# shibatch/rectdetect

Hardware: AMD Instinct MI355X
Metric: 1920x1080 frames/sec (higher is better)
Workload: dtype u8/i32/f32 (bit-exact integer + IEEE f32 stencil path)

## Files before the change

### rectdetect_amd/csrc/rd_k_label.hip

```cpp
#include <stdlib.h>
#include "rd_device.h"
#include "rd_kernels.h"
#include "rd_tidy_tile.h"

namespace {

using namespace rd;

inline int cdiv(int a, int b) { return (a + b - 1) / b; }
const dim3 block2(64, 4);
inline dim3 grid2(int iw, int ih) { return dim3(cdiv(iw, 64), cdiv(ih, 4)); }

#define LT_W 64
#ifndef LT_H
#define LT_H 32
#endif
__device__ __forceinline__ int lt_ld(const int *lab, int a) { return __hip_atomic_load(lab + a, __ATOMIC_RELAXED, __HIP_MEMORY_SCOPE_WORKGROUP); }
__device__ __forceinline__ int lt_find(const int *lab, int a) {
  int l = lt_ld(lab, a);
  while (l != a) { a = l; l = lt_ld(lab, a); }
  return a;
}
__device__ __forceinline__ void lt_union(int *lab, int a, int b) {
  for (;;) {
    a = lt_find(lab, a);
    b = lt_find(lab, b);
    if (a == b) return;
    if (a < b) { const int t = a; a = b; b = t; }
    const int old = atomicMin(&lab[a], b);
    if (old == a) return;
    a = old;
  }
}

#ifndef LT_TY
#define LT_TY 4
#endif
#ifndef LT_TY1
#define LT_TY1 LT_TY
#endif
#define LT_MP 68
template <int SRC, int TY>
__global__ __launch_bounds__(64 * TY) void k_label_tile(int *__restrict__ label, const int *__restrict__ pix, int bgc, int iw, int ih, int *__restrict__ pix_out,
                                                    const float *__restrict__ nms, int *__restrict__ mask0, int *__restrict__ zero_plane, size_t zs, int gdim) {
  constexpr bool BOUNDARY = SRC == 1;
  const rd_tile rd_b = rd_block_tile(gdim);
  if (rd_b.x < 0) return;
  RD_ZSHIFTZ(rd_b.z, zs, label, pix, pix_out, nms, mask0, zero_plane);
  __shared__ int lab[LT_W * LT_H];
  __shared__ int pv[LT_W * LT_H];
  const int tx = threadIdx.x, x = rd_b.x * LT_W + tx, y0 = rd_b.y * LT_H;
  const bool xin = x < iw;
  int v00;
  bool uniform = true;
  int pv8[LT_H / TY];
  if constexpr (SRC == 2) {
    __shared__ __align__(16) uint8_t A[(LT_H + 2 * TD_M) * TD_P], B[(LT_H + 2 * TD_M) * TD_P];
    rect_tidy_tile<LT_H>(A, B, rd_b.x * LT_W, y0, threadIdx.y * 64 + tx, nms, mask0, pix_out, zero_plane, iw, ih, pv8);
    __shared__ int s_t00;
    if (threadIdx.y == 0 && tx == 0) s_t00 = pv8[0];
    __syncthreads();
    v00 = s_t00;
  } else if constexpr (SRC == 3) {
#pragma unroll
    for (int k = 0; k < LT_H / TY; k++) {
      const int y = y0 + threadIdx.y + k * TY;
      const bool in = xin && y < ih;
      const float e = nms[in ? y * iw + x : 0];
      pv8[k] = e > 0.0f ? 1 : 0;
      if (in) { pix_out[y * iw + x] = pv8[k]; zero_plane[y * iw + x] = 0; }
    }
    v00 = nms[(size_t)y0 * iw + rd_b.x * LT_W] > 0.0f ? 1 : 0;
  } else if constexpr (!BOUNDARY) {
    v00 = pix[(size_t)y0 * iw + rd_b.x * LT_W];
#pragma unroll
    for (int k = 0; k < LT_H / TY; k++) {
      const int y = y0 + threadIdx.y + k * TY;
      pv8[k] = pix[(xin && y < ih) ? y * iw + x : 0];
    }
  } else {
    __shared__ int t[(LT_H + 4) * LT_MP];
    __shared__ uint8_t hu[(LT_H + 4) * 64];
    const int x0 = rd_b.x * LT_W, tid = threadIdx.y * 64 + tx;
    const int r00 = pix[(size_t)y0 * iw + x0];
    bool flat = true;
    {
      constexpr int NR = (LT_H + 4 + TY - 1) / TY;
      static_assert(LT_MP == 68 && 4 * (LT_H + 4) <= 64 * TY, "four columns beyond the lanes, one cell per thread");
      int v[NR + 1];
      bool ok[NR + 1];
      const int xl = x0 - 2 + tx;
      const bool cok = xl >= 0 && xl < iw;
#pragma unroll
      for (int i = 0; i < NR; i++) {
        const int r = threadIdx.y + TY * i, yy = y0 - 2 + r;
        ok[i] = r < LT_H + 4 && cok && yy >= 0 && yy < ih;
        v[i] = pix[ok[i] ? yy * iw + xl : 0];
      }
      const int sr = tid >> 2, sc = 64 + (tid & 3);
      {
        const int xx = x0 - 2 + sc, yy = y0 - 2 + sr;
        ok[NR] = sr < LT_H + 4 && xx < iw && yy >= 0 && yy < ih;
        v[NR] = pix[ok[NR] ? yy * iw + xx : 0];
      }
#pragma unroll
      for (int i = 0; i < NR; i++) {
        const int r = threadIdx.y + TY * i;
        if (r < LT_H + 4) { flat = flat && (!ok[i] || v[i] == r00); t[r * LT_MP + tx] = ok[i] ? v[i] : 0; }
      }
      if (sr < LT_H + 4) { flat = flat && (!ok[NR] || v[NR] == r00); t[sr * LT_MP + sc] = ok[NR] ? v[NR] : 0; }
    }
    if (__syncthreads_and(flat)) {
#pragma unroll
      for (int k = 0; k < LT_H / TY; k++) {
        const int y = y0 + threadIdx.y + k * TY;
        if (xin && y < ih) { pix_out[y * iw + x] = -1; label[y * iw + x] = -1; }
      }
      return;
    }
    for (int r = threadIdx.y; r < LT_H + 4; r += TY) {
      const int *row = t + r * LT_MP + tx + 2;
      const int c = row[0];
      hu[r * 64 + tx] = (row[-2] == c && row[-1] == c && row[1] == c && row[2] == c) ? 1 : 0;
    }
    __syncthreads();
#pragma unroll
    for (int k = 0; k < LT_H / TY; k++) {
      const int r = threadIdx.y + k * TY;
      const int y = y0 + r;
      int res = -1;
      if (xin && y < ih && x > 1 && y > 1 && x < iw - 2 && y < ih - 2) {
        const int c0 = t[(r + 2) * LT_MP + tx + 2];
        bool same = true;
#pragma unroll
        for (int dy = 0; dy < 5; dy++) same = same && t[(r + dy) * LT_MP + tx + 2] == c0 && hu[(r + dy) * 64 + tx] != 0;
        if (!same) res = c0;
      }
      pv8[k] = res;
      if (xin && y < ih) pix_out[y * iw + x] = res;
    }
    __shared__ int s_v00;
    if (threadIdx.y == 0 && tx == 0) s_v00 = pv8[0];
    __syncthreads();
    v00 = s_v00;
  }
#pragma unroll
  for (int k = 0; k < LT_H / TY; k++) {
    const int r = threadIdx.y + k * TY;
    const int y = y0 + r;
    const bool valid = xin && y < ih;
    const int v = valid ? pv8[k] : 0;
    uniform = uniform && (!valid || v == v00);
    const int vl = __shfl_up(v, 1);
    const bool lvalid = __shfl_up((int)valid, 1) != 0;
    const bool same = valid && tx > 0 && lvalid && vl == v;
    const unsigned long long starts = __ballot(!same);
    const unsigned long long upto = starts & ((2ull << tx) - 1ull);
    const int start = 63 - __clzll((long long)upto);
    pv[r * LT_W + tx] = v;
    lab[r * LT_W + tx] = (!valid || v == bgc) ? -1 : r * LT_W + start;
  }
  {
    if (__syncthreads_and(uniform)) {
      const int l = v00 == bgc ? -1 : y0 * iw + rd_b.x * LT_W;
#pragma unroll
      for (int r = threadIdx.y; r < LT_H; r += TY) {
        const int y = y0 + r;
        if (xin && y < ih) label[y * iw + x] = l;
      }
      return;
    }
  }
#pragma unroll
  for (int r = threadIdx.y; r < LT_H; r += TY) {
    if (r == 0) continue;
    const int q = r * LT_W + tx;
    if (lab[q] < 0) continue;
    const int v = pv[q];
    const bool wSame = tx > 0 && lab[q - 1] >= 0 && pv[q - 1] == v;
    const bool nSame = lab[q - LT_W] >= 0 && pv[q - LT_W] == v;
    const bool nwSame = tx > 0 && lab[q - LT_W - 1] >= 0 && pv[q - LT_W - 1] == v;
    if (nSame) {
      if (!(wSame && nwSame)) lt_union(lab, q, q - LT_W);
    } else {
      const bool neSame = tx < LT_W - 1 && lab[q - LT_W + 1] >= 0 && pv[q - LT_W + 1] == v;
      const bool eSame = tx < LT_W - 1 && lab[q + 1] >= 0 && pv[q + 1] == v;
      if (nwSame && !wSame) lt_union(lab, q, q - LT_W - 1);
      if (neSame && !eSame) lt_union(lab, q, q - LT_W + 1);
    }
  }
  __syncthreads();
#pragma unroll
  for (int r = threadIdx.y; r < LT_H; r += TY) {
    const int y = y0 + r;
    if (!xin || y >= ih) continue;
    const int q = r * LT_W + tx;
    int l = lab[q];
    if (l >= 0) { l = lt_find(lab, l); l = (y0 + l / LT_W) * iw + rd_b.x * LT_W + l % LT_W; }
    label[y * iw + x] = l;
  }
}

#define LB_SEEN 512
#ifndef LB_DEDUPE
#define LB_DEDUPE 1
#endif
__device__ __forceinline__ void border_union(int *label, int la, int lb, bool want, unsigned long long *seen = nullptr) {
  if (!want) { la = -1; lb = -2; }
  const int pa = __shfl_up(la, 1), pb = __shfl_up(lb, 1);
  bool mine = want && !(__lane_id() > 0 && pa == la && pb == lb);
  if (mine && seen != nullptr) {
    const unsigned long long key = ((unsigned long long)(unsigned)la << 32) | (unsigned)lb;
    unsigned h = ((unsigned)la * 2654435761u ^ (unsigned)lb * 40503u) >> 23;
    for (int probe = 0; probe < 4; probe++) {
      const unsigned long long was = atomicCAS(&seen[h], ~0ull, key);
      if (was == key) { mine = false; break; }
      if (was == ~0ull) break;
      h = (h + 1) & (LB_SEEN - 1);
    }
  }
  if (mine) {
    int a = la, b = lb;
    for (;;) {
      int na = ld_agent(label + a), nb = ld_agent(label + b);
      while (na != a || nb != b) { a = na; b = nb; na = ld_agent(label + a); nb = ld_agent(label + b); }
      if (a == b) break;
      if (a < b) { const int t = a; a = b; b = t; }
      const int old = atomicMin(&label[a], b);
      if (old == a) break;
      a = old;
    }
    const int r = a < b ? a : b;
    if (r < la) atomicMin(&label[la], r);
    if (r < lb) atomicMin(&label[lb], r);
  }
}

__global__ __launch_bounds__(256) void k_label_border(int *label, const int *__restrict__ pix, int bgc, int iw, int ih, int hblocks, size_t zs) {
  RD_ZSHIFT(zs, label, pix);
#if LB_DEDUPE
  __shared__ unsigned long long seen_tab[LB_SEEN];
  for (int i = threadIdx.x; i < LB_SEEN; i += 256) seen_tab[i] = ~0ull;
  __syncthreads();
  unsigned long long *const seen = seen_tab;
#else
  unsigned long long *const seen = nullptr;
#endif
  const bool horizontal = (int)blockIdx.x < hblocks;
  const int t = (horizontal ? blockIdx.x : blockIdx.x - hblocks) * blockDim.x + threadIdx.x;
  if (horizontal) {
    const int nb = (ih - 1) / LT_H;
    const int x = t % iw, k = t / iw;
    const bool in = k < nb;
    const int y = (k + 1) * LT_H;
    const int p = y * iw + x;
    const int v = in ? pix[p] : bgc;
    const bool act = in && v != bgc;
    const bool wSame = act && x > 0 && pix[p - 1] == v;
    const bool nSame = act && pix[p - iw] == v;
    const bool nwSame = act && x > 0 && pix[p - iw - 1] == v;
    const bool neSame = act && x < iw - 1 && pix[p - iw + 1] == v;
    const bool eSame = act && x < iw - 1 && pix[p + 1] == v;
    const int pc = in ? p : 0;
    const int l0 = label[pc], ln = label[in ? p - iw : 0], lnw = label[(in && x > 0) ? p - iw - 1 : 0], lne = label[(in && x < iw - 1) ? p - iw + 1 : 0];
    border_union(label, l0, ln, nSame && !(wSame && nwSame), seen);
    border_union(label, l0, lnw, !nSame && nwSame && !wSame, seen);
    border_union(label, l0, lne, !nSame && neSame && !eSame, seen);
  } else {
    const int nb = (iw - 1) / LT_W;
    const int y = t % ih, k = t / ih;
    const bool in = k < nb;
    const int x = (k + 1) * LT_W;
    const int p = y * iw + x;
    const int v = in ? pix[p] : bgc;
    const bool act = in && v != bgc;
    const bool wSame = act && pix[p - 1] == v;
    const bool nSame = act && y > 0 && pix[p - iw] == v;
    const bool nwSame = act && y > 0 && pix[p - iw - 1] == v;
    const int pc = in ? p : 0;
    const int l0 = label[pc], lw = label[in ? p - 1 : 0], lnw = label[(in && y > 0) ? p - iw - 1 : 0];
    const int ll0 = label[in ? p - 1 : 0], llne = label[(in && y > 0) ? p - 1 - iw + 1 : 0];
    border_union(label, l0, lw, wSame, seen);
    border_union(label, l0, lnw, nwSame && !nSame && !wSame, seen);
    const int pl = p - 1;
    const int vl = in ? pix[pl] : bgc;
    const bool actl = in && vl != bgc && y > 0;
    const bool lne = actl && pix[pl - iw + 1] == vl;
    const bool ln = actl && pix[pl - iw] == vl;
    const bool le = actl && pix[pl + 1] == vl;
    border_union(label, ll0, llne, lne && !ln && !le, seen);
  }
}

__global__ __launch_bounds__(256) void k_label_flatten(int *label, int n, int *vt_table, int *vt_claim, int *vt_list, size_t zs) {
  RD_ZSHIFT(zs, label, vt_table, vt_claim, vt_list);
  const int stride = gridDim.x * blockDim.x;
  for (int i0 = blockIdx.x * blockDim.x + threadIdx.x; i0 < n; i0 += stride * 4) {
    int l[4];
#pragma unroll
    for (int k = 0; k < 4; k++) { const int i = i0 + k * stride; l[k] = i < n ? label[i] : -1; }
    int r[4], n[4];
#pragma unroll
    for (int k = 0; k < 4; k++) { r[k] = l[k] < 0 ? 0 : l[k]; n[k] = l[k] < 0 ? 0 : label[r[k]]; }
    while ((n[0] != r[0]) | (n[1] != r[1]) | (n[2] != r[2]) | (n[3] != r[3])) {
#pragma unroll
      for (int k = 0; k < 4; k++) { r[k] = n[k]; const int v = label[r[k]]; n[k] = l[k] < 0 ? 0 : v; }
    }
#pragma unroll
    for (int k = 0; k < 4; k++)
      if (l[k] >= 0 && r[k] != l[k]) label[i0 + k * stride] = r[k];
  }
  if (vt_list != nullptr && blockIdx.x == 0) {
    const int m = vt_list[0];
    for (int j = threadIdx.x; j < m; j += blockDim.x) {
      const int slot = vt_list[1 + j];
      int *e = vt_table + (size_t)slot * 5;
      e[0] = 0; e[1] = 0; e[2] = 0; e[3] = 0; e[4] = 0;
      vt_claim[slot] = 0x7f7f7f7f;
    }
    __syncthreads();
    if (threadIdx.x == 0) vt_list[0] = 0;
  }
}

#define CS_ROWS 4
#define CS_T 1024
__global__ __launch_bounds__(256) void k_calc_strength(int *out, const float *__restrict__ edge, int *label, int iw, int ih, const int8_t *__restrict__ add, int flatten, size_t zs) {
  RD_ZSHIFT(zs, out, edge, label);
  __shared__ int keys[CS_T], vals[CS_T];
  const int tid = threadIdx.y * 64 + threadIdx.x;
  for (int t = tid; t < CS_T; t += 256) { keys[t] = -1; vals[t] = 0; }
  const int x = blockIdx.x * 64 + threadIdx.x, yb = blockIdx.y * (4 * CS_ROWS) + threadIdx.y;
  int ls[CS_ROWS], as[CS_ROWS];
  float es[CS_ROWS];
#pragma unroll
  for (int k = 0; k < CS_ROWS; k++) {
    const int y = yb + 4 * k;
    const int p = (x < iw && y < ih) ? y * iw + x : 0;
    ls[k] = label[p];
    es[k] = edge[p];
    as[k] = add != nullptr ? add[p] : 0;
  }
  if (flatten) {
    int r[CS_ROWS], n[CS_ROWS];
    bool act[CS_ROWS];
#pragma unroll
    for (int k = 0; k < CS_ROWS; k++) { act[k] = x < iw && yb + 4 * k < ih && ls[k] >= 0; r[k] = act[k] ? ls[k] : 0; }
#pragma unroll
    for (int k = 0; k < CS_ROWS; k++) n[k] = act[k] ? label[r[k]] : 0;
    for (;;) {
      bool moving = false;
#pragma unroll
      for (int k = 0; k < CS_ROWS; k++) moving = moving || n[k] != r[k];
      if (!moving) break;
#pragma unroll
      for (int k = 0; k < CS_ROWS; k++) { r[k] = n[k]; const int v = label[r[k]]; n[k] = act[k] ? v : 0; }
    }
#pragma unroll
    for (int k = 0; k < CS_ROWS; k++)
      if (act[k] && r[k] != ls[k]) { label[(yb + 4 * k) * iw + x] = r[k]; ls[k] = r[k]; }
  }
  __syncthreads();
#pragma unroll
  for (int k = 0; k < CS_ROWS; k++) {
    const int y = yb + 4 * k;
    if (x < iw && y < ih && as[k] != 0) atomicAdd(&out[y * iw + x], as[k]);
    int l = -1, val = 0;
    if (x > 0 && y > 0 && x < iw - 1 && y < ih - 1) {
      l = ls[k];
      if (l > 0) { const float e = es[k]; val = (int)(e * e * 10000.0f); }
    }
    if (l > 0 && val != 0) {
      unsigned h = ((unsigned)l * 2654435761u) >> 22;
      int probes = 0;
      for (;;) {
        const int kprev = atomicCAS(&keys[h], -1, l);
        if (kprev == -1 || kprev == l) { atomicAdd(&vals[h], val); break; }
        h = (h + 1) & (CS_T - 1);
        if (++probes == 32) { atomicAdd(&out[l], val); break; }
      }
    }
  }
  __syncthreads();
  for (int t = tid; t < CS_T; t += 256) if (keys[t] != -1 && vals[t] != 0) atomicAdd(&out[keys[t]], vals[t]);
}

__global__ __launch_bounds__(256) void k_filter_strength(int *label, const int *__restrict__ str, int thre, int iw, int ih) {
  const int x = blockIdx.x * 64 + threadIdx.x, y = blockIdx.y * 4 + threadIdx.y;
  if (x <= 0 || y <= 0 || x >= iw - 1 || y >= ih - 1) return;
  const int p = y * iw + x;
  const int l = label[p];
  if (l <= 0 || str[l] < thre) label[p] = -1;
}

__device__ __forceinline__ void strength_mask_one(int l, int sum, bool interior, int t_edge, int t_strong, int &vs, int &ve, int &lnew) {
  vs = (l > 0 && !(interior && sum < t_strong)) ? 1 : 0;
  ve = (l > 0 && !(interior && sum < t_edge)) ? 1 : 0;
  lnew = (interior && l != -1 && (l <= 0 || sum < t_strong)) ? -1 : l;
}
__device__ __forceinline__ unsigned long long spread4(unsigned long long x) {
  x = (x | (x << 24)) & 0x000000ff000000ffull;
  x = (x | (x << 12)) & 0x000f000f000f000full;
  x = (x | (x << 6)) & 0x0303030303030303ull;
  x = (x | (x << 3)) & 0x1111111111111111ull;
  return x;
}
template <bool VEC>
__global__ __launch_bounds__(256) void k_strength_masks(int *__restrict__ strong, int8_t *__restrict__ strong2, int *__restrict__ edge, int8_t *__restrict__ edge8,
                                                         int *__restrict__ label, const int *__restrict__ str, int t_edge, int t_strong, int iw, int ih, const int8_t *__restrict__ prev,
                                                         unsigned long long *__restrict__ bits) {
  if (VEC) {
    const int x = (blockIdx.x * 64 + threadIdx.x) * 4, y = blockIdx.y * 4 + threadIdx.y;
    if (x >= iw || y >= ih) return;
    const int p = y * iw + x;
    const int4 lv = *(const int4 *)(label + p);
    const int l[4] = { lv.x, lv.y, lv.z, lv.w };
    const bool rowin = y > 0 && y < ih - 1;
    bool interior[4]; int sa[4], sb[4];
#pragma unroll
    for (int k = 0; k < 4; k++) {
      interior[k] = rowin && x + k > 0 && x + k < iw - 1;
      const bool need = l[k] > 0 && interior[k];
      sa[k] = str[need ? l[k] : 0];
      sb[k] = prev ? (int)prev[need ? l[k] : 0] : 0;
    }
    int vs[4], ve[4], ln[4];
#pragma unroll
    for (int k = 0; k < 4; k++) strength_mask_one(l[k], (l[k] > 0 && interior[k]) ? sa[k] + sb[k] : 0, interior[k], t_edge, t_strong, vs[k], ve[k], ln[k]);
    if (strong != nullptr) *(int4 *)(strong + p) = make_int4(vs[0], vs[1], vs[2], vs[3]);
    *(uint32_t *)(strong2 + p) = (uint32_t)vs[0] | ((uint32_t)vs[1] << 8) | ((uint32_t)vs[2] << 16) | ((uint32_t)vs[3] << 24);
    if (bits != nullptr) {
      const unsigned long long b0 = __ballot(vs[0] != 0), b1 = __ballot(vs[1] != 0), b2 = __ballot(vs[2] != 0), b3 = __ballot(vs[3] != 0);
      const int j = threadIdx.x;
      const int wx = blockIdx.x * 4 + j, wpr = (iw + 63) >> 6;
      if (j < 4 && wx < wpr) {
        const int sh = 16 * j;
        bits[(size_t)y * wpr + wx] = spread4((b0 >> sh) & 0xffffull) | (spread4((b1 >> sh) & 0xffffull) << 1) | (spread4((b2 >> sh) & 0xffffull) << 2) | (spread4((b3 >> sh) & 0xffffull) << 3);
      }
    }
    if (edge != nullptr) *(int4 *)(edge + p) = make_int4(ve[0], ve[1], ve[2], ve[3]);
    *(uint32_t *)(edge8 + p) = (uint32_t)ve[0] | ((uint32_t)ve[1] << 8) | ((uint32_t)ve[2] << 16) | ((uint32_t)ve[3] << 24);
    if (ln[0] != l[0] || ln[1] != l[1] || ln[2] != l[2] || ln[3] != l[3]) *(int4 *)(label + p) = make_int4(ln[0], ln[1], ln[2], ln[3]);
    return;
  }
  const int x = blockIdx.x * 64 + threadIdx.x, y = blockIdx.y * 4 + threadIdx.y;
  if (x >= iw || y >= ih) return;
  const int p = y * iw + x;
  const int l = label[p];
  const bool interior = x > 0 && y > 0 && x < iw - 1 && y < ih - 1;
  const int sum = (l > 0 && interior) ? str[l] + (prev ? (int)prev[l] : 0) : 0;
  int vs, ve, ln;
  strength_mask_one(l, sum, interior, t_edge, t_strong, vs, ve, ln);
  if (bits != nullptr) { const unsigned long long m = __ballot(vs != 0); if (threadIdx.x == 0) bits[(size_t)y * ((iw + 63) >> 6) + blockIdx.x] = m; }
  if (strong != nullptr) strong[p] = vs;
  strong2[p] = (int8_t)vs;
  if (edge != nullptr) edge[p] = ve;
  edge8[p] = (int8_t)ve;
  if (ln != l) label[p] = ln;
}

__device__ int strong_before(const int *label0, const int *str0, const int8_t *ring0, size_t zs, int zz, int q, int iw, int ih, int t_strong) {
  for (;;) {
    if (zz < 0) return (int)ring0[q];
    const int l2 = ld_agent((const int *)((const char *)label0 + (size_t)zz * zs + (size_t)q * 4));
    if (l2 <= 0) return 0;
    const int qy = q / iw, qx = q - qy * iw;
    if (!(qx > 0 && qy > 0 && qx < iw - 1 && qy < ih - 1)) return 1;
    const int s2 = *(const int *)((const char *)str0 + (size_t)zz * zs + (size_t)l2 * 4);
    if (s2 >= t_strong) return 1;
    if (s2 + 1 < t_strong) return 0;
    q = l2; zz--;
  }
}
__global__ __launch_bounds__(256) void k_strength_masks_group(int8_t *ring, int8_t *__restrict__ edge8, int *label, const int *__restrict__ str, int t_edge, int t_strong,
                                                               int iw, int ih, unsigned long long *__restrict__ bits, long t0, int nring, size_t zs) {
  const int z = blockIdx.z;
  const int *label0 = label, *str0 = str;
  const size_t N = (size_t)iw * ih;
  const int8_t *ring0 = ring + (size_t)(t0 % nring) * N;
  int8_t *out = ring + (size_t)((t0 + z + 1) % nring) * N;
  RD_ZSHIFT(zs, edge8, label, str, bits);
  const int x = (blockIdx.x * 64 + threadIdx.x) * 4, y = blockIdx.y * 4 + threadIdx.y;
  if (x >= iw || y >= ih) return;
  const int p = y * iw + x;
  const int4 lv = *(const int4 *)(label + p);
  const int l[4] = { lv.x, lv.y, lv.z, lv.w };
  const bool rowin = y > 0 && y < ih - 1;
  bool interior[4], need[4]; int sa[4], sb[4];
  bool ask = false;
#pragma unroll
  for (int k = 0; k < 4; k++) {
    interior[k] = rowin && x + k > 0 && x + k < iw - 1;
    need[k] = l[k] > 0 && interior[k];
    sa[k] = str[need[k] ? l[k] : 0];
  }
#pragma unroll
  for (int k = 0; k < 4; k++) { sb[k] = 0; ask = ask || (need[k] && (sa[k] == t_strong - 1 || sa[k] == t_edge - 1)); }
  if (__any(ask)) {
#pragma unroll
    for (int k = 0; k < 4; k++) if (need[k] && (sa[k] == t_strong - 1 || sa[k] == t_edge - 1)) sb[k] = strong_before(label0, str0, ring0, zs, z - 1, l[k], iw, ih, t_strong);
  }
  int vs[4], ve[4], ln[4];
#pragma unroll
  for (int k = 0; k < 4; k++) strength_mask_one(l[k], need[k] ? sa[k] + sb[k] : 0, interior[k], t_edge, t_strong, vs[k], ve[k], ln[k]);
  *(uint32_t *)(out + p) = (uint32_t)vs[0] | ((uint32_t)vs[1] << 8) | ((uint32_t)vs[2] << 16) | ((uint32_t)vs[3] << 24);
  {
    const unsigned long long b0 = __ballot(vs[0] != 0), b1 = __ballot(vs[1] != 0), b2 = __ballot(vs[2] != 0), b3 = __ballot(vs[3] != 0);
    const int j = threadIdx.x;
    const int wx = blockIdx.x * 4 + j, wpr = (iw + 63) >> 6;
    if (j < 4 && wx < wpr) {
      const int sh = 16 * j;
      bits[(size_t)y * wpr + wx] = spread4((b0 >> sh) & 0xffffull) | (spread4((b1 >> sh) & 0xffffull) << 1) | (spread4((b2 >> sh) & 0xffffull) << 2) | (spread4((b3 >> sh) & 0xffffull) << 3);
    }
  }
  *(uint32_t *)(edge8 + p) = (uint32_t)ve[0] | ((uint32_t)ve[1] << 8) | ((uint32_t)ve[2] << 16) | ((uint32_t)ve[3] << 24);
  if (ln[0] != l[0] || ln[1] != l[1] || ln[2] != l[2] || ln[3] != l[3]) *(int4 *)(label + p) = make_int4(ln[0], ln[1], ln[2], ln[3]);
}

__global__ __launch_bounds__(256) void k_poly_mask_bits(unsigned long long *__restrict__ bits, const int *__restrict__ label, const int *__restrict__ str, int thre, int iw, int ih, size_t zs) {
  RD_ZSHIFT(zs, bits, label, str);
  const int x = blockIdx.x * 64 + threadIdx.x, y = blockIdx.y * 4 + threadIdx.y;
  if (y >= ih) return;
  bool on = false;
  if (x < iw) {
    const int l = label[y * iw + x];
    const bool interior = x > 0 && y > 0 && x < iw - 1 && y < ih - 1;
    on = l > 0 && (!interior || str[l] >= thre);
  }
  const unsigned long long m = __ballot(on);
  if (threadIdx.x == 0) bits[(size_t)y * ((iw + 63) >> 6) + blockIdx.x] = m;
}

}

namespace rdk {

int strength_masks_group_fits(int iw, const void *label, const void *ring, const void *edge8, size_t zs) {
  return (iw & 3) == 0 && (((uintptr_t)label | zs) & 15) == 0 && (((uintptr_t)ring | (uintptr_t)edge8) & 3) == 0;
}
void strength_masks_group(hipStream_t s, int8_t *ring, int8_t *edge8, int *label, const int *str, int t_edge, int t_strong, int iw, int ih, unsigned long long *bits, long t0, int nring, int nz, size_t zs) {
  hipLaunchKernelGGL(k_strength_masks_group, dim3(cdiv(iw, 256), cdiv(ih, 4), nz), block2, 0, s, ring, edge8, label, str, t_edge, t_strong, iw, ih, bits, t0, nring, zs);
}

void label8(hipStream_t s, int *label, const int *pix, int bgc, int iw, int ih, int skip_flatten) {
  const size_t zs = 0;
  hipLaunchKernelGGL((k_label_tile<0, LT_TY>), dim3(rd_tile_blocks(cdiv(iw, LT_W), cdiv(ih, LT_H), 1)), dim3(64, LT_TY), 0, s, label, pix, bgc, iw, ih, (int *)nullptr, (const float *)nullptr, (int *)nullptr, (int *)nullptr, zs, rd_gdim(cdiv(iw, LT_W), cdiv(ih, LT_H), 1));
  const int nh = ((ih - 1) / LT_H) * iw, nv = ((iw - 1) / LT_W) * ih;
  const int hb = cdiv(nh, 256), vb = cdiv(nv, 256);
  if (hb + vb > 0) hipLaunchKernelGGL(k_label_border, dim3(hb + vb), dim3(256), 0, s, label, pix, bgc, iw, ih, hb, zs);
  if (skip_flatten) return;
  const int n = iw * ih;
  int g = cdiv(n, 256 * 4);
  hipLaunchKernelGGL(k_label_flatten, dim3(g < 1 ? 1 : g), dim3(256), 0, s, label, n, (int *)nullptr, (int *)nullptr, (int *)nullptr, zs);
}

void label8_tidy(hipStream_t s, int *label, int *mask0, int *tidy, const float *nms, int *zero_plane, int iw, int ih, int skip_flatten, int nz, size_t zs) {
  hipLaunchKernelGGL((k_label_tile<2, 4>), dim3(rd_tile_blocks(cdiv(iw, LT_W), cdiv(ih, LT_H), nz)), dim3(64, 4), 0, s, label, (const int *)nullptr, -1, iw, ih, tidy, nms, mask0, zero_plane, zs, rd_gdim(cdiv(iw, LT_W), cdiv(ih, LT_H), nz));
  const int nh = ((ih - 1) / LT_H) * iw, nv = ((iw - 1) / LT_W) * ih;
  const int hb = cdiv(nh, 256), vb = cdiv(nv, 256);
  if (vb > 0) hipLaunchKernelGGL(k_label_border, dim3(vb, 1, nz), dim3(256), 0, s, label, (const int *)tidy, -1, iw, ih, 0, zs);
  if (hb > 0) hipLaunchKernelGGL(k_label_border, dim3(hb, 1, nz), dim3(256), 0, s, label, (const int *)tidy, -1, iw, ih, hb, zs);
  if (skip_flatten) return;
  const int n = iw * ih;
  int g = cdiv(n, 256 * 4);
  hipLaunchKernelGGL(k_label_flatten, dim3(g < 1 ? 1 : g, 1, nz), dim3(256), 0, s, label, n, (int *)nullptr, (int *)nullptr, (int *)nullptr, zs);
}

void label8_positive(hipStream_t s, int *label, int *mask, const float *nms, int *zero_plane, int iw, int ih, int skip_flatten, int nz, size_t zs) {
  hipLaunchKernelGGL((k_label_tile<3, LT_TY>), dim3(rd_tile_blocks(cdiv(iw, LT_W), cdiv(ih, LT_H), nz)), dim3(64, LT_TY), 0, s, label, (const int *)nullptr, 0, iw, ih, mask, nms, (int *)nullptr, zero_plane, zs, rd_gdim(cdiv(iw, LT_W), cdiv(ih, LT_H), nz));
  const int nh = ((ih - 1) / LT_H) * iw, nv = ((iw - 1) / LT_W) * ih;
  const int hb = cdiv(nh, 256), vb = cdiv(nv, 256);
  if (hb + vb > 0) hipLaunchKernelGGL(k_label_border, dim3(hb + vb, 1, nz), dim3(256), 0, s, label, (const int *)mask, 0, iw, ih, hb, zs);
  if (skip_flatten) return;
  const int n = iw * ih;
  int g = cdiv(n, 256 * 4);
  hipLaunchKernelGGL(k_label_flatten, dim3(g < 1 ? 1 : g, 1, nz), dim3(256), 0, s, label, n, (int *)nullptr, (int *)nullptr, (int *)nullptr, zs);
}

void poly_mask_bits(hipStream_t s, unsigned long long *bits, const int *label, const int *str, int thre, int iw, int ih, int nz, size_t zs) {
  hipLaunchKernelGGL(k_poly_mask_bits, dim3(cdiv(iw, 64), cdiv(ih, 4), nz), block2, 0, s, bits, label, str, thre, iw, ih, zs);
}

void label8_boundary(hipStream_t s, int *label, int *marks, const int *region, int iw, int ih, int *vt_table, int *vt_claim, int *vt_list, int nz, size_t zs, int flatten) {
  hipLaunchKernelGGL((k_label_tile<1, LT_TY1>), dim3(rd_tile_blocks(cdiv(iw, LT_W), cdiv(ih, LT_H), nz)), dim3(64, LT_TY1), 0, s, label, region, -1, iw, ih, marks, (const float *)nullptr, (int *)nullptr, (int *)nullptr, zs, rd_gdim(cdiv(iw, LT_W), cdiv(ih, LT_H), nz));
  const int nh = ((ih - 1) / LT_H) * iw, nv = ((iw - 1) / LT_W) * ih;
  const int hb = cdiv(nh, 256), vb = cdiv(nv, 256);
  if (hb + vb > 0) hipLaunchKernelGGL(k_label_border, dim3(hb + vb, 1, nz), dim3(256), 0, s, label, (const int *)marks, -1, iw, ih, hb, zs);
  const int n = iw * ih;
  int g = flatten ? cdiv(n, 256 * 4) : 1;
  hipLaunchKernelGGL(k_label_flatten, dim3(g < 1 ? 1 : g, 1, nz), dim3(256), 0, s, label, flatten ? n : 0, vt_table, vt_claim, vt_list, zs);
}
void label8_flatten(hipStream_t s, int *label, int n) {
  int g = cdiv(n, 256 * 4);
  hipLaunchKernelGGL(k_label_flatten, dim3(g < 1 ? 1 : g), dim3(256), 0, s, label, n, (int *)nullptr, (int *)nullptr, (int *)nullptr, (size_t)0);
}

void calc_strength(hipStream_t s, int *out, const float *edge, int *label, int iw, int ih, const int8_t *add, int flatten, int nz, size_t zs) {
  hipLaunchKernelGGL(k_calc_strength, dim3(cdiv(iw, 64), cdiv(ih, 4 * CS_ROWS), nz), block2, 0, s, out, edge, label, iw, ih, add, flatten, zs);
}

void strength_masks(hipStream_t s, int *strong, int8_t *strong2, int *edge, int8_t *edge8, int *label, const int *str, int t_edge, int t_strong, int iw, int ih, const int8_t *prev, unsigned long long *bits) {
  const bool vec = (iw & 3) == 0 && ((((uintptr_t)strong | (uintptr_t)label | (uintptr_t)edge) & 15) == 0) && ((((uintptr_t)strong2 | (uintptr_t)edge8) & 3) == 0);
  if (vec) hipLaunchKernelGGL(k_strength_masks<true>, dim3(cdiv(iw, 256), cdiv(ih, 4)), block2, 0, s, strong, strong2, edge, edge8, label, str, t_edge, t_strong, iw, ih, prev, bits);
  else hipLaunchKernelGGL(k_strength_masks<false>, grid2(iw, ih), block2, 0, s, strong, strong2, edge, edge8, label, str, t_edge, t_strong, iw, ih, prev, bits);
}

void filter_strength(hipStream_t s, int *label, const int *str, int thre, int iw, int ih) {
  hipLaunchKernelGGL(k_filter_strength, grid2(iw, ih), block2, 0, s, label, str, thre, iw, ih);
}

}
```

### rectdetect_amd/csrc/rd_tidy_tile.h

```cpp
#pragma once
#include "rd_device.h"

namespace rd {

struct bitrow { unsigned long long lo, hi; };
__device__ __forceinline__ bitrow br(unsigned long long lo, unsigned long long hi) { bitrow r; r.lo = lo; r.hi = hi; return r; }
__device__ __forceinline__ bitrow operator&(bitrow a, bitrow b) { return br(a.lo & b.lo, a.hi & b.hi); }
__device__ __forceinline__ bitrow operator|(bitrow a, bitrow b) { return br(a.lo | b.lo, a.hi | b.hi); }
__device__ __forceinline__ bitrow operator~(bitrow a) { return br(~a.lo, ~a.hi); }
__device__ __forceinline__ bitrow br_west(bitrow a) { return br(a.lo << 1, (a.hi << 1) | (a.lo >> 63)); }
__device__ __forceinline__ bitrow br_east(bitrow a) { return br((a.lo >> 1) | (a.hi << 63), a.hi >> 1); }
__device__ __forceinline__ int br_bit(bitrow a, int b) { return (int)(((b < 64 ? a.lo >> b : a.hi >> (b - 64))) & 1ull); }
__device__ __forceinline__ bitrow br_range(int first, int last) {
  if (first < 0) first = 0;
  if (last > 127) last = 127;
  if (first > last) return br(0, 0);
  const unsigned long long lo = first < 64 ? ((~0ull << first) & (last >= 63 ? ~0ull : ((1ull << (last + 1)) - 1ull))) : 0ull;
  const int f2 = first < 64 ? 0 : first - 64, l2 = last - 64;
  const unsigned long long hi = l2 < 0 ? 0ull : ((~0ull << f2) & (l2 >= 63 ? ~0ull : ((1ull << (l2 + 1)) - 1ull)));
  return br(lo, hi);
}
__device__ __forceinline__ void br_count8(bitrow u, bitrow m, bitrow d, bitrow &ge1, bitrow &ge2) {
  const bitrow in[8] = { br_west(u), u, br_east(u), br_west(m), br_east(m), br_west(d), d, br_east(d) };
  ge1 = br(0, 0); ge2 = br(0, 0);
#pragma unroll
  for (int k = 0; k < 8; k++) { ge2 = ge2 | (ge1 & in[k]); ge1 = ge1 | in[k]; }
}

#define TD_M 4
#define TD_P (64 + 2 * TD_M)
template <int ROWS>
__device__ __forceinline__ void rect_tidy_tile(uint8_t *A, uint8_t *B, int x0, int y0, int tid, const float *__restrict__ nms, int *__restrict__ mask0, int *__restrict__ tidy,
                                               int *__restrict__ zero_plane, int iw, int ih, int (&outv)[ROWS / 4]) {
  constexpr int R = ROWS + 2 * TD_M;
  static_assert(R * 3 * (int)sizeof(bitrow) <= R * TD_P, "three bit planes per byte buffer");
  bitrow *M = (bitrow *)A, *NZ = M + R, *E2 = NZ + R;
  bitrow *O = (bitrow *)B, *T0 = O + R;
  const int lane = tid & 63, w = tid >> 6;
  {
    constexpr int RW = (R + 3) / 4;
    float fa[RW], fb[RW];
    bool oka[RW], okb[RW];
#pragma unroll
    for (int k = 0; k < RW; k++) {
      const int r = w + 4 * k, y = y0 - TD_M + r;
      const int xa = x0 - TD_M + lane, xb = x0 - TD_M + 64 + lane;
      const bool rowin = r < R && y >= 0 && y < ih;
      oka[k] = rowin && xa >= 0 && xa < iw;
      okb[k] = rowin && lane < 8 && xb < iw;
      fa[k] = nms[oka[k] ? y * iw + xa : 0];
      fb[k] = nms[okb[k] ? y * iw + xb : 0];
    }
#pragma unroll
    for (int k = 0; k < RW; k++) {
      const int r = w + 4 * k, y = y0 - TD_M + r;
      const bool va = oka[k] && fa[k] > 0.0f, vb = okb[k] && fb[k] > 0.0f;
      const unsigned long long ba = __ballot(va), bb = __ballot(vb);
      if (r < R && lane == 0) M[r] = br(ba, bb);
      const int ta = lane - TD_M, tb = lane + 64 - TD_M, tr = r - TD_M;
      if (mask0 != nullptr && tr >= 0 && tr < ROWS) {
        if (oka[k] && ta >= 0) mask0[y * iw + x0 + ta] = va ? 1 : 0;
        if (okb[k] && tb < 64) mask0[y * iw + x0 + tb] = vb ? 1 : 0;
      }
    }
  }
  __syncthreads();
  const int r = tid;
  const int y = y0 - TD_M + r;
  const bitrow in1 = (y >= 1 && y <= ih - 2) ? br_range(1 - x0 + TD_M, iw - 2 - x0 + TD_M) : br(0, 0);
  const bitrow in2 = (y >= 2 && y <= ih - 3) ? br_range(2 - x0 + TD_M, iw - 3 - x0 + TD_M) : br(0, 0);
  const unsigned long long even = (((x0 - TD_M + y) & 1) == 0) ? 0x5555555555555555ull : 0xaaaaaaaaaaaaaaaaull;
  if (r >= 1 && r < R - 1) {
    bitrow ge1, ge2;
    br_count8(M[r - 1], M[r], M[r + 1], ge1, ge2);
    const bitrow on = M[r] & in1;
    NZ[r] = on & ge1;
    E2[r] = on & ge1 & ~ge2;
  } else if (r < R) { NZ[r] = br(0, 0); E2[r] = br(0, 0); }
  __syncthreads();
  if (r >= 2 && r < R - 2) {
    const bitrow zn = NZ[r - 1], zm = NZ[r], zs = NZ[r + 1], en = E2[r - 1], em = E2[r], es = E2[r + 1];
    const bitrow pat = (br_west(em) & br_east(zm)) | (br_west(zm) & br_east(em)) | (en & zs) | (zn & es) |
                       (br_west(en) & br_east(es)) | (br_east(en) & br_west(es)) |
                       (br_east(em) & br_west(es)) | (br_west(em) & br_east(es)) | (br_east(en) & es) | (br_west(en) & es);
    O[r] = in2 & (zm | pat);
  } else if (r < R) O[r] = br(0, 0);
  __syncthreads();
  if (r >= 3 && r < R - 3) {
    const bitrow o = O[r];
    const bitrow kill = in1 & br(even, even) & (O[r - 1] | O[r + 1]) & (br_west(o) | br_east(o));
    T0[r] = o & ~kill;
  } else if (r < R) T0[r] = br(0, 0);
  __syncthreads();
  bitrow *T1 = E2;
  if (r >= TD_M && r < R - TD_M) {
    const bitrow o = T0[r];
    const bitrow kill = in1 & br(~even, ~even) & (T0[r - 1] | T0[r + 1]) & (br_west(o) | br_east(o));
    T1[r] = o & ~kill;
  }
  __syncthreads();
  const int tx = lane, x = x0 + tx;
#pragma unroll
  for (int j = 0; j < ROWS / 4; j++) {
    const int tr = w + 4 * j, yy = y0 + tr;
    int v = 0;
    if (x < iw && yy < ih) {
      v = br_bit(T1[tr + TD_M], tx + TD_M);
      tidy[yy * iw + x] = v;
      if (zero_plane) zero_plane[yy * iw + x] = 0;
    }
    outv[j] = v;
  }
}

}
```

Before: 3046.

## Assign contiguous row strips per wave and compute union pairs in registers via DPP

```diff
diff --git a/rectdetect_amd/csrc/rd_k_label.hip b/rectdetect_amd/csrc/rd_k_label.hip
--- a/rectdetect_amd/csrc/rd_k_label.hip
+++ b/rectdetect_amd/csrc/rd_k_label.hip
@@ -15,7 +15,10 @@
 #ifndef LT_H
 #define LT_H 32
 #endif
+#define LT_NIL (LT_W * LT_H)
 __device__ __forceinline__ int lt_ld(const int *lab, int a) { return __hip_atomic_load(lab + a, __ATOMIC_RELAXED, __HIP_MEMORY_SCOPE_WORKGROUP); }
+__device__ __forceinline__ int lt_west(int v) { return __builtin_amdgcn_update_dpp(v, v, 0x138, 0xf, 0xf, false); }
+__device__ __forceinline__ int lt_east(int v) { return __builtin_amdgcn_update_dpp(v, v, 0x130, 0xf, 0xf, false); }
 __device__ __forceinline__ int lt_find(const int *lab, int a) {
   int l = lt_ld(lab, a);
   while (l != a) { a = l; l = lt_ld(lab, a); }
@@ -31,6 +34,12 @@
     if (old == a) return;
     a = old;
   }
+}
+__device__ __forceinline__ void lt_pairs(bool act, bool wok, bool eok, int v, int vW, int vE, int vP, int vPW, int vPE, int sP, int sPW, int sPE, int &pA, int &pB) {
+  const bool wSame = wok && vW == v, eSame = eok && vE == v, nSame = vP == v, nwSame = wok && vPW == v, neSame = eok && vPE == v;
+  const bool goA = act && (nSame ? !(wSame && nwSame) : (nwSame && !wSame));
+  pA = goA ? (nSame ? sP : sPW) : LT_NIL;
+  pB = (act && !nSame && neSame && !eSame) ? sPE : LT_NIL;
 }
 
 #ifndef LT_TY
@@ -44,44 +53,51 @@
 __global__ __launch_bounds__(64 * TY) void k_label_tile(int *__restrict__ label, const int *__restrict__ pix, int bgc, int iw, int ih, int *__restrict__ pix_out,
                                                     const float *__restrict__ nms, int *__restrict__ mask0, int *__restrict__ zero_plane, size_t zs, int gdim) {
   constexpr bool BOUNDARY = SRC == 1;
+  constexpr int RW = LT_H / TY;
+  static_assert(RW * TY == LT_H, "whole strips");
   const rd_tile rd_b = rd_block_tile(gdim);
   if (rd_b.x < 0) return;
   RD_ZSHIFTZ(rd_b.z, zs, label, pix, pix_out, nms, mask0, zero_plane);
-  __shared__ int lab[LT_W * LT_H];
-  __shared__ int pv[LT_W * LT_H];
-  const int tx = threadIdx.x, x = rd_b.x * LT_W + tx, y0 = rd_b.y * LT_H;
+  __shared__ int lab[LT_W * LT_H + 1];
+  __shared__ int s_pv[TY * LT_W], s_st[TY * LT_W];
+  const int tx = threadIdx.x, wv = rd_ty(), x = rd_b.x * LT_W + tx, y0 = rd_b.y * LT_H, r0 = wv * RW;
   const bool xin = x < iw;
   int v00;
   bool uniform = true;
-  int pv8[LT_H / TY];
+  int pv8[RW];
   if constexpr (SRC == 2) {
     __shared__ __align__(16) uint8_t A[(LT_H + 2 * TD_M) * TD_P], B[(LT_H + 2 * TD_M) * TD_P];
-    rect_tidy_tile<LT_H>(A, B, rd_b.x * LT_W, y0, threadIdx.y * 64 + tx, nms, mask0, pix_out, zero_plane, iw, ih, pv8);
+    static_assert(TY == 4, "rect_tidy_tile: four waves");
+    rect_tidy_tile<LT_H>(A, B, rd_b.x * LT_W, y0, wv * 64 + tx, nms, mask0, pix_out, zero_plane, iw, ih, pv8);
     __shared__ int s_t00;
-    if (threadIdx.y == 0 && tx == 0) s_t00 = pv8[0];
+    if (wv == 0 && tx == 0) s_t00 = pv8[0];
     __syncthreads();
     v00 = s_t00;
   } else if constexpr (SRC == 3) {
-#pragma unroll
-    for (int k = 0; k < LT_H / TY; k++) {
-      const int y = y0 + threadIdx.y + k * TY;
-      const bool in = xin && y < ih;
-      const float e = nms[in ? y * iw + x : 0];
-      pv8[k] = e > 0.0f ? 1 : 0;
-      if (in) { pix_out[y * iw + x] = pv8[k]; zero_plane[y * iw + x] = 0; }
+    float e[RW];
+#pragma unroll
+    for (int k = 0; k < RW; k++) {
+      const int y = y0 + r0 + k;
+      e[k] = nms[(xin && y < ih) ? y * iw + x : 0];
+    }
+#pragma unroll
+    for (int k = 0; k < RW; k++) {
+      const int y = y0 + r0 + k;
+      pv8[k] = e[k] > 0.0f ? 1 : 0;
+      if (xin && y < ih) { pix_out[y * iw + x] = pv8[k]; zero_plane[y * iw + x] = 0; }
     }
     v00 = nms[(size_t)y0 * iw + rd_b.x * LT_W] > 0.0f ? 1 : 0;
   } else if constexpr (!BOUNDARY) {
     v00 = pix[(size_t)y0 * iw + rd_b.x * LT_W];
 #pragma unroll
-    for (int k = 0; k < LT_H / TY; k++) {
-      const int y = y0 + threadIdx.y + k * TY;
+    for (int k = 0; k < RW; k++) {
+      const int y = y0 + r0 + k;
       pv8[k] = pix[(xin && y < ih) ? y * iw + x : 0];
     }
   } else {
     __shared__ int t[(LT_H + 4) * LT_MP];
     __shared__ uint8_t hu[(LT_H + 4) * 64];
-    const int x0 = rd_b.x * LT_W, tid = threadIdx.y * 64 + tx;
+    const int x0 = rd_b.x * LT_W, tid = wv * 64 + tx;
     const int r00 = pix[(size_t)y0 * iw + x0];
     bool flat = true;
     {
@@ -93,7 +109,7 @@
       const bool cok = xl >= 0 && xl < iw;
 #pragma unroll
       for (int i = 0; i < NR; i++) {
-        const int r = threadIdx.y + TY * i, yy = y0 - 2 + r;
+        const int r = wv + TY * i, yy = y0 - 2 + r;
         ok[i] = r < LT_H + 4 && cok && yy >= 0 && yy < ih;
         v[i] = pix[ok[i] ? yy * iw + xl : 0];
       }
@@ -105,99 +121,111 @@
       }
 #pragma unroll
       for (int i = 0; i < NR; i++) {
-        const int r = threadIdx.y + TY * i;
+        const int r = wv + TY * i;
         if (r < LT_H + 4) { flat = flat && (!ok[i] || v[i] == r00); t[r * LT_MP + tx] = ok[i] ? v[i] : 0; }
       }
       if (sr < LT_H + 4) { flat = flat && (!ok[NR] || v[NR] == r00); t[sr * LT_MP + sc] = ok[NR] ? v[NR] : 0; }
     }
     if (__syncthreads_and(flat)) {
 #pragma unroll
-      for (int k = 0; k < LT_H / TY; k++) {
-        const int y = y0 + threadIdx.y + k * TY;
+      for (int k = 0; k < RW; k++) {
+        const int y = y0 + r0 + k;
         if (xin && y < ih) { pix_out[y * iw + x] = -1; label[y * iw + x] = -1; }
       }
       return;
     }
-    for (int r = threadIdx.y; r < LT_H + 4; r += TY) {
+    for (int r = wv; r < LT_H + 4; r += TY) {
       const int *row = t + r * LT_MP + tx + 2;
       const int c = row[0];
       hu[r * 64 + tx] = (row[-2] == c && row[-1] == c && row[1] == c && row[2] == c) ? 1 : 0;
     }
     __syncthreads();
-#pragma unroll
-    for (int k = 0; k < LT_H / TY; k++) {
-      const int r = threadIdx.y + k * TY;
-      const int y = y0 + r;
+    int cc[RW + 4];
+    bool hh[RW + 4];
+#pragma unroll
+    for (int i = 0; i < RW + 4; i++) { cc[i] = t[(r0 + i) * LT_MP + tx + 2]; hh[i] = hu[(r0 + i) * 64 + tx] != 0; }
+#pragma unroll
+    for (int k = 0; k < RW; k++) {
+      const int y = y0 + r0 + k;
       int res = -1;
-      if (xin && y < ih && x > 1 && y > 1 && x < iw - 2 && y < ih - 2) {
-        const int c0 = t[(r + 2) * LT_MP + tx + 2];
-        bool same = true;
-#pragma unroll
-        for (int dy = 0; dy < 5; dy++) same = same && t[(r + dy) * LT_MP + tx + 2] == c0 && hu[(r + dy) * 64 + tx] != 0;
-        if (!same) res = c0;
-      }
+      const int c0 = cc[k + 2];
+      bool same = true;
+#pragma unroll
+      for (int dy = 0; dy < 5; dy++) same = same && cc[k + dy] == c0 && hh[k + dy];
+      if (xin && y < ih && x > 1 && y > 1 && x < iw - 2 && y < ih - 2 && !same) res = c0;
       pv8[k] = res;
       if (xin && y < ih) pix_out[y * iw + x] = res;
     }
     __shared__ int s_v00;
-    if (threadIdx.y == 0 && tx == 0) s_v00 = pv8[0];
+    if (wv == 0 && tx == 0) s_v00 = pv8[0];
     __syncthreads();
     v00 = s_v00;
   }
-#pragma unroll
-  for (int k = 0; k < LT_H / TY; k++) {
-    const int r = threadIdx.y + k * TY;
+  const bool wok = tx > 0, eok = tx < LT_W - 1 && x + 1 < iw;
+  int st[RW], pA[RW], pB[RW];
+  int v0 = 0, v0W = 0, v0E = 0;
+  int vP = 0, vPW = 0, vPE = 0, sP = LT_NIL, sPW = LT_NIL, sPE = LT_NIL;
+#pragma unroll
+  for (int k = 0; k < RW; k++) {
+    const int r = r0 + k;
     const int y = y0 + r;
     const bool valid = xin && y < ih;
     const int v = valid ? pv8[k] : 0;
     uniform = uniform && (!valid || v == v00);
-    const int vl = __shfl_up(v, 1);
-    const bool lvalid = __shfl_up((int)valid, 1) != 0;
-    const bool same = valid && tx > 0 && lvalid && vl == v;
+    const int vW = lt_west(v), vE = lt_east(v);
+    const bool same = valid && wok && vW == v;
     const unsigned long long starts = __ballot(!same);
     const unsigned long long upto = starts & ((2ull << tx) - 1ull);
     const int start = 63 - __clzll((long long)upto);
-    pv[r * LT_W + tx] = v;
-    lab[r * LT_W + tx] = (!valid || v == bgc) ? -1 : r * LT_W + start;
-  }
+    const bool act = valid && v != bgc;
+    const int s = act ? r * LT_W + start : LT_NIL;
+    lab[r * LT_W + tx] = act ? s : -1;
+    st[k] = s;
+    const int sW = lt_west(s), sE = lt_east(s);
+    if (k == 0) { v0 = v; v0W = vW; v0E = vE; }
+    else lt_pairs(act, wok, eok, v, vW, vE, vP, vPW, vPE, sP, sPW, sPE, pA[k], pB[k]);
+    vP = v; vPW = vW; vPE = vE; sP = s; sPW = sW; sPE = sE;
+  }
+  s_pv[wv * LT_W + tx] = vP;
+  s_st[wv * LT_W + tx] = sP;
+  if (wv == 0 && tx == 0) lab[LT_NIL] = LT_NIL;
   {
     if (__syncthreads_and(uniform)) {
       const int l = v00 == bgc ? -1 : y0 * iw + rd_b.x * LT_W;
 #pragma unroll
-      for (int r = threadIdx.y; r < LT_H; r += TY) {
-        const int y = y0 + r;
+      for (int k = 0; k < RW; k++) {
+        const int y = y0 + r0 + k;
         if (xin && y < ih) label[y * iw + x] = l;
       }
       return;
     }
   }
-#pragma unroll
-  for (int r = threadIdx.y; r < LT_H; r += TY) {
-    if (r == 0) continue;
-    const int q = r * LT_W + tx;
-    if (lab[q] < 0) continue;
-    const int v = pv[q];
-    const bool wSame = tx > 0 && lab[q - 1] >= 0 && pv[q - 1] == v;
-    const bool nSame = lab[q - LT_W] >= 0 && pv[q - LT_W] == v;
-    const bool nwSame = tx > 0 && lab[q - LT_W - 1] >= 0 && pv[q - LT_W - 1] == v;
-    if (nSame) {
-      if (!(wSame && nwSame)) lt_union(lab, q, q - LT_W);
-    } else {
-      const bool neSame = tx < LT_W - 1 && lab[q - LT_W + 1] >= 0 && pv[q - LT_W + 1] == v;
-      const bool eSame = tx < LT_W - 1 && lab[q + 1] >= 0 && pv[q + 1] == v;
-      if (nwSame && !wSame) lt_union(lab, q, q - LT_W - 1);
-      if (neSame && !eSame) lt_union(lab, q, q - LT_W + 1);
-    }
+  if (wv > 0) {
+    vP = s_pv[(wv - 1) * LT_W + tx];
+    sP = s_st[(wv - 1) * LT_W + tx];
+    lt_pairs(st[0] != LT_NIL, wok, eok, v0, v0W, v0E, vP, lt_west(vP), lt_east(vP), sP, lt_west(sP), lt_east(sP), pA[0], pB[0]);
+  } else { pA[0] = LT_NIL; pB[0] = LT_NIL; }
+#pragma unroll
+  for (int k = 0; k < RW; k++) {
+    if (pA[k] != LT_NIL) lt_union(lab, st[k], pA[k]);
+    if (pB[k] != LT_NIL) lt_union(lab, st[k], pB[k]);
   }
   __syncthreads();
-#pragma unroll
-  for (int r = threadIdx.y; r < LT_H; r += TY) {
-    const int y = y0 + r;
-    if (!xin || y >= ih) continue;
-    const int q = r * LT_W + tx;
-    int l = lab[q];
-    if (l >= 0) { l = lt_find(lab, l); l = (y0 + l / LT_W) * iw + rd_b.x * LT_W + l % LT_W; }
-    label[y * iw + x] = l;
+  int rt[RW], nx[RW];
+#pragma unroll
+  for (int k = 0; k < RW; k++) { rt[k] = st[k]; nx[k] = lt_ld(lab, rt[k]); }
+  for (;;) {
+    bool moving = false;
+#pragma unroll
+    for (int k = 0; k < RW; k++) moving = moving || nx[k] != rt[k];
+    if (!moving) break;
+#pragma unroll
+    for (int k = 0; k < RW; k++) { rt[k] = nx[k]; nx[k] = lt_ld(lab, rt[k]); }
+  }
+#pragma unroll
+  for (int k = 0; k < RW; k++) {
+    const int y = y0 + r0 + k;
+    if (xin && y < ih) label[y * iw + x] = st[k] == LT_NIL ? -1 : (y0 + rt[k] / LT_W) * iw + rd_b.x * LT_W + rt[k] % LT_W;
   }
 }
 
diff --git a/rectdetect_amd/csrc/rd_tidy_tile.h b/rectdetect_amd/csrc/rd_tidy_tile.h
--- a/rectdetect_amd/csrc/rd_tidy_tile.h
+++ b/rectdetect_amd/csrc/rd_tidy_tile.h
@@ -102,7 +102,7 @@
   const int tx = lane, x = x0 + tx;
 #pragma unroll
   for (int j = 0; j < ROWS / 4; j++) {
-    const int tr = w + 4 * j, yy = y0 + tr;
+    const int tr = (ROWS / 4) * w + j, yy = y0 + tr;
     int v = 0;
     if (x < iw && yy < ih) {
       v = br_bit(T1[tr + TD_M], tx + TD_M);
```

Result: faster. 3155, median of 6 (+3.6%).
